# unilight/seq2seq-vc

Hardware: AMD Instinct MI355X
Metric: mel-frames/sec (train) (higher is better)
Workload: dtype bf16; 1 GPU; VTN egs/arctic/vc1 (vtn.v1.yaml) training step: fwd+Seq2SeqLoss+bwd+clip+Adam+WarmupLR; batch_per_gpu=32, global_batch=32, T_src=256, T_tgt=256, mel_dim=80, parallelism=dp1, split_backward=False, hip_graph=True, backward_stages=1

## Files before the change

include/s2svc_hip.h:

```cpp
#ifndef S2SVC_HIP_H
#define S2SVC_HIP_H
#include <stdint.h>
#ifdef __cplusplus
extern "C" {
#endif

const char* s2svc_last_error(void);
int s2svc_abi_version(void);
int s2svc_launch_floor(int workgroups, int threads, void* sink_1024_words, void* stream);

int s2svc_event_create(void** out );
int s2svc_event_destroy(void* ev);
int s2svc_event_record(void* ev, void* stream);
int s2svc_stream_wait_event(void* stream, void* ev);

enum { S2SVC_LAYOUT_KC = 0,
       S2SVC_LAYOUT_RC = 1 };
enum { S2SVC_OP_DENSE = 0,
       S2SVC_OP_CONV1D = 1,
       S2SVC_OP_CONV2D_S2 = 2,
       S2SVC_OP_TCONV2D_S2 = 3 };

typedef struct {
  const void* ptr;
// ... 18 lines not shown
  const void* res;
  int64_t ldr, rbs0, rbs1;
  int32_t M, N, K;
  int32_t nb0, nb1;
  int32_t act;
  float alpha;
  int32_t dtype;
  int32_t accumulate;
  int32_t splitk;
  float* ws;
  float* a_rowsum;
  float* a_rowsum_ws;
  int32_t a_rowsum_accumulate;
  int32_t tile_hint;
  const void* emask;
  int64_t ldm;
  float drop_p;
  int32_t emask_mode;
  const uint64_t* seed_base;
  uint64_t seed_off;
  int32_t c_map;
  int32_t cm_T1, cm_F1, cm_Tc, cm_Fc, cm_pt, cm_pf;
  int32_t reserved3_;
  void* c_pre;
} s2svc_gemm_desc;

int s2svc_gemm(const s2svc_gemm_desc* desc , void* stream);
const char* s2svc_gemm_last_route(void);

int s2svc_tconv2d_weights(int O, int C, const float* w, void* out_bf16, void* stream);

int s2svc_gemm_grouped_ok(const s2svc_gemm_desc* desc );
int s2svc_gemm_grouped(const s2svc_gemm_desc* descs , int n, int tile, void* stream);
int s2svc_gemm_grouped_batched(const s2svc_gemm_desc* descs , int n, void* stream);
int s2svc_gemm_wgrad_ok(const s2svc_gemm_desc* desc );
int64_t s2svc_gemm_wgrad_ws_floats(const s2svc_gemm_desc* descs , int n);
int s2svc_gemm_wgrad_grouped(const s2svc_gemm_desc* descs , int n, float* ws, void* stream);
int s2svc_gemm_wgrad_grouped_bg(const s2svc_gemm_desc* descs , int n, float* ws, void* stream, int wgs_cap);
int s2svc_gemm_set_w8(int on, int kt_chunk);

int s2svc_gemm_set_8ph(int mode);

int s2svc_layernorm_fwd(int dtype, int rows, int D, const void* x, const void* res, float drop_p, float hscale,
                        const uint64_t* seed_base, uint64_t seed_off, const float* gamma, const float* beta, float eps,
                        void* y, void* s_out, float* mean, float* rstd, void* stream);
int s2svc_layernorm_bwd(int dtype, int rows, int D, const void* dy, const void* s, const float* mean, const float* rstd,
                        const float* gamma, const void* ds_extra, float drop_p, float hscale, const uint64_t* seed_base,
                        uint64_t seed_off, void* ds, void* dh, void* stream);
int s2svc_colreduce(int dtype, int rows, int D, int mode, const void* dy, const void* x, const float* mean,
                    const float* rstd, float scale, float* out_sum, float* out_dot, int accumulate, float* ws,
                    int ws_chunks, int Tn, const int32_t* vlens , void* stream);
typedef struct {
  const void* dy;
  const void* x;
  const float* mean;
  const float* rstd;
  float* out_sum;
  float* out_dot;
  float* ws;
  int32_t dtype, rows, D, mode, accumulate, ws_chunks;
  float scale;
  int32_t reserved_;
} s2svc_colreduce_item;
int s2svc_colreduce_grouped(const s2svc_colreduce_item* items , int n, void* stream);
int s2svc_layernorm_bwd_pg_chunks(int dtype, int rows, int D, const void* dy, const void* s, const float* gamma, const void* ds_extra,
                                  const void* ds, const void* dh);
// ... 374 lines not shown
```

seq2seq_vc_amd/csrc/gemm_8ph.hip:

```cpp
#include <cstring>
#include "gemm_common.h"
#include "lds_dma.h"

namespace {

enum { P8_DENSE = 0, P8_CONV2D = 1, P8_TCONV2D = 2, P8_CONV1D = 3 };

template <int BM, int BN, bool GROUPED = false>
__device__ __forceinline__ void p8_tile_of_block(int& bm, int& bn) {
  const int gx = gridDim.x, gy = gridDim.y, nwg = gx * gy;
  int id = blockIdx.y * gx + blockIdx.x;
  if (gridDim.z == 1 || (nwg & 7) == 0) id = xcd_contiguous_id(id, nwg);
  if (GROUPED && gx >= 4) {
    const int qe = (nwg >> 3) < 32 ? (nwg >> 3) : 32;
    const int t2 = 2 * qe * BN / BM;
    int gh = 1;
    while (gh * 2 <= gy && 4 * gh * gh <= t2) gh *= 2;
    const int per = gh * gx, grp = id / per, within = id - grp * per;
    const int rows = (gy - grp * gh) < gh ? (gy - grp * gh) : gh;
    const int c = within / rows;
    bm = grp * gh + (within - c * rows);
    bn = c;
    return;
  }
  bm = id / gx;
  bn = id - bm * gx;
}

template <int KIND>
struct P8Walk {
  int kt, c0, kh, kw;
  __device__ __forceinline__ void init(const s2svc_operand& o, int kt0) {
    kt = kt0;
    if (KIND == P8_CONV1D) {
      const int ntap = 2 * o.pad + 1;
      const int cs = kt0 / ntap;
      c0 = cs * 64;
      kh = kt0 - cs * ntap;
      kw = 0;
    }
    if (KIND == P8_CONV2D) {
      const int cs = kt0 / 9, tap = kt0 - cs * 9;
      c0 = cs * 64;
      kh = tap / 3;
      kw = tap - kh * 3;
    }
    if (KIND == P8_TCONV2D) {
      const int nf = 2 - (o.pad & 1), ntap = (2 - (o.pad >> 1)) * nf;
      const int cs = kt0 / ntap, tap = kt0 - cs * ntap;
      c0 = cs * 64;
      kh = tap / nf;
      kw = tap - kh * nf;
    }
  }
  __device__ __forceinline__ int64_t off_bytes(const s2svc_operand& o) const {
    if (KIND == P8_CONV2D) return ((int64_t)(kh * o.F1 + kw) * o.ld + c0) * 2;
    if (KIND == P8_TCONV2D) return (-(int64_t)(kh * o.F2 + kw) * o.ld + c0) * 2;
    if (KIND == P8_CONV1D) return ((int64_t)(kh - o.pad) * o.ld + c0) * 2;
    return (int64_t)kt * 128;
  }
  __device__ __forceinline__ int64_t off_bytes_b(const s2svc_operand& o) const {
    if (KIND == P8_CONV2D) return ((int64_t)(kh * 3 + kw) * o.C + c0) * 2;
    if (KIND == P8_TCONV2D) return ((int64_t)(kh * (2 - (o.pad & 1)) + kw) * o.C + c0) * 2;
    if (KIND == P8_CONV1D) return ((int64_t)kh * o.C + c0) * 2;
    return (int64_t)kt * 128;
  }
  __device__ __forceinline__ int bit() const { return KIND == P8_CONV1D ? 1 << kh : 1 << (2 * kh + kw); }
  __device__ __forceinline__ void next(const s2svc_operand& o) {
    ++kt;
    if (KIND == P8_CONV2D) {
      if (++kw == 3) {
        kw = 0;
        if (++kh == 3) {
          kh = 0;
          c0 += 64;
        }
      }
    }
    if (KIND == P8_CONV1D) {
      if (++kh == 2 * o.pad + 1) {
        kh = 0;
        c0 += 64;
      }
    }
    if (KIND == P8_TCONV2D) {
      if (++kw == 2 - (o.pad & 1)) {
        kw = 0;
        if (++kh == 2 - (o.pad >> 1)) {
          kh = 0;
          c0 += 64;
        }
      }
    }
  }
};

template <int KIND>
__device__ __forceinline__ uint32_t p8_rowoff(const s2svc_operand& o, int r, int R, int c) {
  if (r >= R) r = R - 1;
  int64_t e;
  if (KIND == P8_CONV2D) {
    const int bt = r / o.F2, f2 = r - bt * o.F2;
    const int b = bt / o.T2, t2 = bt - b * o.T2;
    e = ((int64_t)(b * o.T1 + 2 * t2) * o.F1 + 2 * f2) * o.ld;
  } else if (KIND == P8_TCONV2D) {
    const int per_b = o.T1 * o.F1;
    const int b = r / per_b, rem = r - b * per_b;
    const int i = rem / o.F1, j = rem - i * o.F1;
    e = ((int64_t)(b * o.T2 + i) * o.F2 + j) * o.ld;
  } else {
    e = (int64_t)r * o.ld;
  }
  return (uint32_t)((e + c * 8) * 2);
}

__device__ __forceinline__ int p8_rowmask(const s2svc_operand& o, int r, int R) {
  if (r >= R) return 0;
  const int per_b = o.T1 * o.F1;
  const int rem = r - (r / per_b) * per_b;
  const int i = rem / o.F1, j = rem - i * o.F1;
  int m = 0;
#pragma unroll
  for (int ta = 0; ta < 2; ++ta)
#pragma unroll
    for (int fb = 0; fb < 2; ++fb)
      if (i - ta >= 0 && i - ta < o.T2 && j - fb >= 0 && j - fb < o.F2) m |= 1 << (2 * ta + fb);
  return m;
}

__device__ __forceinline__ int p8_rowmask1d(const s2svc_operand& o, int r, int R) {
  if (r >= R) return 0;
  const int t = r - (r / o.T) * o.T;
  int m = 0;
  for (int tap = 0; tap <= 2 * o.pad; ++tap)
    if (t + tap - o.pad >= 0 && t + tap - o.pad < o.T) m |= 1 << tap;
  return m;
}
template <int KA>
__device__ __forceinline__ int p8_rowmask_of(const s2svc_operand& o, int r, int R) {
  return KA == P8_TCONV2D ? p8_rowmask(o, r, R) : KA == P8_CONV1D ? p8_rowmask1d(o, r, R) : 0;
}

template <int NI>
__device__ __forceinline__ void p8_issue(const char* base, const uint32_t (&off)[NI], char* lds_unit, int wave_s) {
  const char* b = base ? base : reinterpret_cast<const char*>(&g_zero16);
#pragma unroll
  for (int e = 0; e < NI; ++e) {
    const uint32_t o = base ? off[e] : 0u;
    __builtin_amdgcn_global_load_lds((gbl_void*)(b + o), (lds_void*)(lds_unit + (wave_s * NI + e) * 1024), 16, 0, 0);
  }
}

template <int NI>
__device__ __forceinline__ void p8_issue_masked(const char* base, const uint32_t (&off)[NI], const int (&mask)[NI], int bit,
                                                char* lds_unit, int wave_s) {
  const char* z = reinterpret_cast<const char*>(&g_zero16);
#pragma unroll
  for (int e = 0; e < NI; ++e) {
    const char* src = (base && (mask[e] & bit)) ? base + off[e] : z;
    __builtin_amdgcn_global_load_lds((gbl_void*)src, (lds_void*)(lds_unit + (wave_s * NI + e) * 1024), 16, 0, 0);
  }
}

template <int KA, int NI>
__device__ __forceinline__ void p8_issue_a(const char* base, const uint32_t (&off)[NI], const int (&mask)[NI], int bit, char* lds_unit,
                                           int wave_s) {
  if (KA == P8_TCONV2D || KA == P8_CONV1D) p8_issue_masked<NI>(base, off, mask, bit, lds_unit, wave_s);
  else p8_issue<NI>(base, off, lds_unit, wave_s);
}

template <int NF>
__device__ __forceinline__ void p8_read(const char* unit, int rd_base, int p0, int p1, bf16x8_t (&f)[NF][2]) {
#pragma unroll
  for (int i = 0; i < NF; ++i) {
    f[i][0] = *reinterpret_cast<const bf16x8_t*>(unit + rd_base + i * 2048 + p0);
    f[i][1] = *reinterpret_cast<const bf16x8_t*>(unit + rd_base + i * 2048 + p1);
  }
}

template <int NA, int NB>
__device__ __forceinline__ void p8_mfma(const bf16x8_t (&a)[NA][2], const bf16x8_t (&b)[NB][2], f32x4_t (&acc)[NA][NB]) {
  __builtin_amdgcn_s_setprio(1);
#pragma unroll
  for (int ks = 0; ks < 2; ++ks)
#pragma unroll
    for (int i = 0; i < NA; ++i)
#pragma unroll
      for (int j = 0; j < NB; ++j) acc[i][j] = __builtin_amdgcn_mfma_f32_16x16x32_bf16(a[i][ks], b[j][ks], acc[i][j], 0, 0, 0);
  __builtin_amdgcn_s_setprio(0);
}

#define P8_PHASE_SYNC_IN()                 \
  wait_lgkm0();                         \
  __builtin_amdgcn_sched_barrier(0);       \
  __builtin_amdgcn_s_barrier();            \
  __builtin_amdgcn_sched_barrier(0)
#define P8_PHASE_SYNC_OUT()                \
  __builtin_amdgcn_sched_barrier(0);       \
  __builtin_amdgcn_s_barrier();            \
  __builtin_amdgcn_sched_barrier(0)

template <int KA, int WR, int WC, bool STAGGER, bool LEAN = false>
__global__ __launch_bounds__(512) void gemm_8ph_kernel_q(const s2svc_gemm_desc d) {
  static_assert(WR * WC == 8 && (WC == 2 || WC == 4), "8 waves");
  constexpr int BM = WR * 128, BN = WC * 64;
  constexpr int NIA = WR, NIB = WC / 2;
  constexpr int UA = WR * 64 * 128, UB = WC * 32 * 128;
  constexpr int BUF = 2 * UA + 2 * UB;
  constexpr int OA0 = 0, OA1 = UA, OB0 = 2 * UA, OB1 = 2 * UA + UB;
  __shared__ __attribute__((aligned(1024))) char smem[2 * BUF];
  const int zb = blockIdx.z;
  const int z0 = zb / d.nb1, z1 = zb - z0 * d.nb1;
  int tile_m, tile_n;
  p8_tile_of_block<BM, BN, true>(tile_m, tile_n);
  const int m0 = tile_m * BM, n0 = tile_n * BN;
  const char* Ab = reinterpret_cast<const char*>((const bf16_t*)d.A.ptr + (int64_t)z0 * d.A.bs0 + (int64_t)z1 * d.A.bs1);
  const char* Bb = reinterpret_cast<const char*>((const bf16_t*)d.B.ptr + (int64_t)z0 * d.B.bs0 + (int64_t)z1 * d.B.bs1);
  const int nt = d.K / 64;
  const int lane = threadIdx.x & 63;
  const int wave = __builtin_amdgcn_readfirstlane(threadIdx.x >> 6);
  const int wr = wave / WC, wc = wave % WC;
  const int half = wave >> 2;
  const int lr = lane & 15, lg = lane >> 4;

  uint32_t offA[2][NIA], offB[2][NIB];
  int mA[2][NIA];
#pragma unroll
  for (int e = 0; e < NIA; ++e) {
    const int ru = (wave * NIA + e) * 8 + (lane >> 3);
    const int c = (lane & 7) ^ ((ru >> 1) & 7);
#pragma unroll
    for (int h = 0; h < 2; ++h) {
      const int row = m0 + (ru >> 6) * 128 + h * 64 + (ru & 63);
      offA[h][e] = p8_rowoff<KA>(d.A, row, d.M, c);
      mA[h][e] = p8_rowmask_of<KA>(d.A, row, d.M);
    }
  }
#pragma unroll
  for (int e = 0; e < NIB; ++e) {
    const int ru = (wave * NIB + e) * 8 + (lane >> 3);
    const int c = (lane & 7) ^ ((ru >> 1) & 7);
#pragma unroll
    for (int h = 0; h < 2; ++h) offB[h][e] = p8_rowoff<P8_DENSE>(d.B, n0 + (ru >> 5) * 64 + h * 32 + (ru & 31), d.N, c);
  }
  const int sw = (lr >> 1) & 7;
  const int p0 = (lg ^ sw) << 4, p1 = ((4 + lg) ^ sw) << 4;
  const int rdA = (wr * 64 + lr) * 128, rdB = (wc * 32 + lr) * 128;
// ... 39 lines not shown
    char* oth = smem + ((t & 1) ^ 1) * BUF;
    const char* a2 = (t + 2 < nt) ? Ab + wa.off_bytes(d.A) : nullptr;
    const int bit2 = wa.bit();
    const char* b2 = (t + 2 < nt) ? Bb + wa.off_bytes_b(d.A) : nullptr;
    const char* b1 = (t + 1 < nt) ? Bb + wb.off_bytes_b(d.A) : nullptr;
    p8_read<2>(cur + OB0, rdB, p0, p1, fb0);
    p8_read<4>(cur + OA0, rdA, p0, p1, fa);
    p8_issue<NIB>(b1, offB[0], oth + OB0, wave);
    P8_PHASE_SYNC_IN();
    p8_mfma<4, 2>(fa, fb0, acc[0][0]);
    P8_PHASE_SYNC_OUT();
    p8_read<2>(cur + OB1, rdB, p0, p1, fb1);
    p8_issue_a<KA, NIA>(a2, offA[0], mA[0], bit2, cur + OA0, wave);
    P8_PHASE_SYNC_IN();
    p8_mfma<4, 2>(fa, fb1, acc[0][1]);
    P8_PHASE_SYNC_OUT();
    p8_read<4>(cur + OA1, rdA, p0, p1, fa);
    p8_issue<NIB>(b2, offB[1], cur + OB1, wave);
    P8_PHASE_SYNC_IN();
    p8_mfma<4, 2>(fa, fb1, acc[1][1]);
    P8_PHASE_SYNC_OUT();
    p8_issue_a<KA, NIA>(a2, offA[1], mA[1], bit2, cur + OA1, wave);
    wait_vmcnt<2 * NIA + NIB>();
    P8_PHASE_SYNC_IN();
    p8_mfma<4, 2>(fa, fb0, acc[1][0]);
    P8_PHASE_SYNC_OUT();
    wa.next(d.A);
    wb.next(d.A);
  }
  if (STAGGER && half == 0) __builtin_amdgcn_s_barrier();
  wait_vmcnt<0>();
  __syncthreads();
  float* cs = reinterpret_cast<float*>(smem) + wave * (64 * 32);
  const bool cmap_lean = KA == P8_TCONV2D && d.tile_hint != 65 && epilogue_cmap_ok(d);
  const c_map_t cmq = c_map_make(d);
#pragma unroll 1
  for (int q = 0; q < 4; ++q) {
    switch (q) {
      case 0: epilogue_stage<64, 32>(acc[0][0], cs); break;
      case 1: epilogue_stage<64, 32>(acc[0][1], cs); break;
      case 2: epilogue_stage<64, 32>(acc[1][0], cs); break;
      default: epilogue_stage<64, 32>(acc[1][1], cs); break;
    }
    if (LEAN) epilogue_flush_common<64, 32>(d, m0 + wr * 128 + (q >> 1) * 64, n0 + wc * 64 + (q & 1) * 32, cs);
    else if (KA == P8_TCONV2D && cmap_lean) epilogue_flush_cmap<64, 32>(d, cmq, m0 + wr * 128 + (q >> 1) * 64, n0 + wc * 64 + (q & 1) * 32, cs);
    else epilogue_flush<64, 32>(d, z0, z1, m0 + wr * 128 + (q >> 1) * 64, n0 + wc * 64 + (q & 1) * 32, cs, 1, 0, zb);
  }
}

template <int KA, bool STAGGER, int LEAN = 0>
__global__ __launch_bounds__(512) void gemm_8ph_kernel_128(const s2svc_gemm_desc d) {
  constexpr int UNIT = 16384, BUF = 3 * UNIT;
  __shared__ __attribute__((aligned(1024))) char smem[2 * BUF];
  const int zb = blockIdx.z;
  const int z0 = zb / d.nb1, z1 = zb - z0 * d.nb1;
  int tile_m, tile_n;
  p8_tile_of_block<256, 128>(tile_m, tile_n);
  const int m0 = tile_m * 256, n0 = tile_n * 128;
  const char* Ab = reinterpret_cast<const char*>((const bf16_t*)d.A.ptr + (int64_t)z0 * d.A.bs0 + (int64_t)z1 * d.A.bs1);
  const char* Bb = reinterpret_cast<const char*>((const bf16_t*)d.B.ptr + (int64_t)z0 * d.B.bs0 + (int64_t)z1 * d.B.bs1);
  const int nt = d.K / 64;
  const int lane = threadIdx.x & 63;
  const int wave = __builtin_amdgcn_readfirstlane(threadIdx.x >> 6);
  const int wr = wave >> 2, wc = wave & 3;
  const int lr = lane & 15, lg = lane >> 4;

  uint32_t offA[2][2], offB[2];
  int mA[2][2];
#pragma unroll
  for (int e = 0; e < 2; ++e) {
    const int ru = (wave * 2 + e) * 8 + (lane >> 3);
    const int c = (lane & 7) ^ ((ru >> 1) & 7);
#pragma unroll
    for (int h = 0; h < 2; ++h) {
      const int row = m0 + (ru >> 6) * 128 + h * 64 + (ru & 63);
      offA[h][e] = p8_rowoff<KA>(d.A, row, d.M, c);
      mA[h][e] = p8_rowmask_of<KA>(d.A, row, d.M);
    }
// ... 819 lines not shown
    if (md >= 2) { if (md == 2 || md == 2 + ph) return ph; continue; }
    if (t <= 256 && t >= 224 && (geo == 0 || tiles < 224 || tiles > 256)) return ph;
  }
  return 0;
}

int g_p8_geo = -1;
int p8_force_bn() {
  if (g_p8_geo < 0) g_p8_geo = 0;
  return g_p8_geo;
}

bool p8_operand_ok(const s2svc_operand& o, int rows, int K) {
  if (o.layout != S2SVC_LAYOUT_KC || ((uintptr_t)o.ptr) % 16 || o.ld % 8 || o.bs0 % 8 || o.bs1 % 8) return false;
  int64_t elems;
  if (o.mode == S2SVC_OP_DENSE) {
    elems = (int64_t)rows * o.ld;
  } else if (o.mode == S2SVC_OP_CONV2D_S2) {
    if (o.C % 64 || o.C < 64 || K != 9 * o.C) return false;
    elems = (int64_t)(rows / (o.T2 * o.F2) + 1) * o.T1 * o.F1 * o.ld;
  } else if (o.mode == S2SVC_OP_CONV1D) {
    if (o.pad < 0 || o.pad > 7 || o.C % 64 || o.C < 64 || K != (2 * o.pad + 1) * o.C || o.T <= 0 || rows % o.T || o.ld < o.C) return false;
    elems = (int64_t)(rows + o.pad) * o.ld;
  } else if (o.mode == S2SVC_OP_TCONV2D_S2) {
    const int ntap = (2 - (o.pad >> 1)) * (2 - (o.pad & 1));
    if (o.pad < 0 || o.pad > 3 || o.C % 64 || o.C < 64 || K != ntap * o.C || o.T1 <= 0 || o.F1 <= 0) return false;
    elems = (int64_t)(rows / (o.T1 * o.F1) + 1) * o.T2 * o.F2 * o.ld;
  } else {
    return false;
  }
  return elems * 2 < (1ll << 32);
}

}

extern "C" int s2svc_gemm_set_8ph(int mode) {
  const int prev = p8_mode() | (p8_force_bn() << 4) | ((p8_n96_mode() + 1) << 8);
  if (mode >= 0) {
    const int n96 = (mode >> 8) & 15;
    mode &= 255;
    if ((mode & 15) <= 2 && (mode >> 4) <= 3) {
      g_p8_mode = mode & 15;
      g_p8_geo = mode >> 4;
    }
    if (n96 >= 1 && n96 <= 6) g_p8_n96 = n96 - 1;
  }
  return prev;
}

extern "C" int s2svc_gemm_try_8ph(const s2svc_gemm_desc* desc, void* stream) {
  const s2svc_gemm_desc& d = *desc;
  const int mode = p8_mode();
  if (mode != 0 && d.tile_hint != 64 && p8_tr_ok(d) && (int64_t)(d.M / 256) * (d.N / 128) >= p8_min_tiles()) {
    const int64_t t128 = (int64_t)(d.M / 256) * (d.N / 128);
    if (p8_tr_take_q(d.N % 256 == 0, t128 / 2, t128)) {
      dim3 grid((unsigned)(d.N / 256), (unsigned)(d.M / 256), 1);
      s2s_gemm_route(mode == 2 ? "8ph_tr_q<noskew>" : "8ph_tr_q<skew>");
      if (mode == 2) hipLaunchKernelGGL((gemm_8ph_tr_kernel_q<false>), grid, dim3(512), 0, (hipStream_t)stream, d);
      else hipLaunchKernelGGL((gemm_8ph_tr_kernel_q<true>), grid, dim3(512), 0, (hipStream_t)stream, d);
    } else {
      dim3 grid((unsigned)(d.N / 128), (unsigned)(d.M / 256), 1);
      s2s_gemm_route(mode == 2 ? "8ph_tr<noskew>" : "8ph_tr<skew>");
      if (mode == 2) hipLaunchKernelGGL((gemm_8ph_tr_kernel<false>), grid, dim3(512), 0, (hipStream_t)stream, d);
      else hipLaunchKernelGGL((gemm_8ph_tr_kernel<true>), grid, dim3(512), 0, (hipStream_t)stream, d);
    }
    S2S_CHECK_LAUNCH("gemm_8ph_tr_kernel");
    return 1;
  }
  if (mode == 0 || d.dtype != S2S_BF16 || d.splitk > 1 || d.a_rowsum || d.tile_hint == 64) return 0;
  if (d.K < 128 || d.K % 64 || d.M < 256 || d.N < 64) return 0;
  if (d.B.mode != S2SVC_OP_DENSE || !p8_operand_ok(d.A, d.M, d.K) || !p8_operand_ok(d.B, d.N, d.K)) return 0;
  if (d.A.mode == S2SVC_OP_TCONV2D_S2 && d.nb0 * d.nb1 != 1) return 0;
  const int64_t nb = (int64_t)d.nb0 * d.nb1;
  const int64_t t256 = (int64_t)((d.M + 255) / 256) * ((d.N + 255) / 256) * nb;
  const int64_t t512 = (int64_t)((d.M + 511) / 512) * ((d.N + 127) / 128) * nb;
  const int64_t t128 = (int64_t)((d.M + 255) / 256) * ((d.N + 127) / 128) * nb;
  int geo = 0;
  const int waste256 = (int)(((d.N + 255) / 256) * 256 - d.N), waste128 = (int)(((d.N + 127) / 128) * 128 - d.N);
  const double cost256 = 2.0 * 0.85 * (double)((t256 + 255) / 256), cost128 = (double)((t128 + 255) / 256);
  if (waste256 <= waste128 && t256 >= 192 && cost256 <= cost128) geo = 1;
  else if (d.M >= 2048 && t512 >= 160 && t512 <= 256) geo = 2;
  else if (t128 >= p8_min_tiles()) geo = 3;
  if (p8_force_bn() >= 1 && p8_force_bn() <= 3) geo = p8_force_bn();
  hipStream_t st = (hipStream_t)stream;
  if (d.A.mode == S2SVC_OP_DENSE && nb == 1 && mode == 1 && (p8_force_bn() == 0 || p8_n96_mode() >= 2) && epilogue_common_ok(d)) {
    const int ph = p8_n96_phases(d, geo, geo == 1 ? t256 : geo == 2 ? t512 : t128);
    if (ph) {
      dim3 grid((unsigned)((d.N + 96 * ph - 1) / (96 * ph)), (unsigned)((d.M + 255) / 256), 1);
      s2s_gemm_route(ph == 3 ? "8ph_n96<3>" : "8ph_n96<2>");
      if (ph == 3) hipLaunchKernelGGL((gemm_8ph_kernel_n96<3, true>), grid, dim3(512), 0, st, d);
      else hipLaunchKernelGGL((gemm_8ph_kernel_n96<2, true>), grid, dim3(512), 0, st, d);
      S2S_CHECK_LAUNCH("gemm_8ph_kernel_n96");
      return 1;
    }
  }
  if (geo == 0) return 0;
  if (d.A.mode == S2SVC_OP_CONV1D) {
    if (mode != 1 || nb != 1 || !epilogue_common_ok(d)) return 0;
    const int bm1 = geo == 2 ? 512 : 256, bn1 = geo == 1 ? 256 : 128;
    dim3 grid1((unsigned)((d.N + bn1 - 1) / bn1), (unsigned)((d.M + bm1 - 1) / bm1), 1);
    s2s_gemm_route(geo == 1 ? "8ph_q<CONV1D,2,4>" : geo == 2 ? "8ph_q<CONV1D,4,2>" : "8ph_128<CONV1D,lean>");
    if (geo == 1) hipLaunchKernelGGL((gemm_8ph_kernel_q<P8_CONV1D, 2, 4, true, true>), grid1, dim3(512), 0, st, d);
    else if (geo == 2) hipLaunchKernelGGL((gemm_8ph_kernel_q<P8_CONV1D, 4, 2, true, true>), grid1, dim3(512), 0, st, d);
    else hipLaunchKernelGGL((gemm_8ph_kernel_128<P8_CONV1D, true, 1>), grid1, dim3(512), 0, st, d);
    S2S_CHECK_LAUNCH("gemm_8ph_kernel (conv1d)");
    return 1;
  }
  const bool conv = d.A.mode == S2SVC_OP_CONV2D_S2, tconv = d.A.mode == S2SVC_OP_TCONV2D_S2;
  const int bm = geo == 2 ? 512 : 256, bn = geo == 1 ? 256 : 128;
  dim3 grid((unsigned)((d.N + bn - 1) / bn), (unsigned)((d.M + bm - 1) / bm), (unsigned)nb);
#define P8_LAUNCH(PRE, POST, KERNEL, ...)                                                                   \
  do {                                                                                                    \
    s2s_gemm_route(mode == 2 ? (conv ? PRE "CONV2D" POST ",noskew>" : tconv ? PRE "TCONV2D" POST ",noskew>" : PRE "DENSE" POST ",noskew>")    \
                             : (conv ? PRE "CONV2D" POST ",skew>" : tconv ? PRE "TCONV2D" POST ",skew>" : PRE "DENSE" POST ",skew>"));        \
    if (mode == 2) {                                                                                      \
      if (conv) hipLaunchKernelGGL((KERNEL<P8_CONV2D, ##__VA_ARGS__, false>), grid, dim3(512), 0, st, d); \
      else if (tconv) hipLaunchKernelGGL((KERNEL<P8_TCONV2D, ##__VA_ARGS__, false>), grid, dim3(512), 0, st, d); \
      else hipLaunchKernelGGL((KERNEL<P8_DENSE, ##__VA_ARGS__, false>), grid, dim3(512), 0, st, d);       \
    } else {                                                                                              \
// ... 24 lines not shown
  group_args g;
  std::memset(&g, 0, sizeof(g));
  int64_t t128 = 0, t256 = 0;
  bool all256 = true;
  int mask = 0, m = 0;
  for (int i = 0; i < n; ++i) {
    if (!p8_tr_ok(descs[i]) || (int64_t)(descs[i].M / 128) * (descs[i].N / 128) < 64) continue;
    mask |= 1 << i;
    g.d[m++] = descs[i];
    t128 += (int64_t)(descs[i].M / 256) * (descs[i].N / 128);
    all256 = all256 && descs[i].N % 256 == 0;
    t256 += (int64_t)(descs[i].M / 256) * (descs[i].N / 256);
  }
  if (m == 0) return 0;
  S2S_REQUIRE(t128 < (1ll << 30), "gemm_grouped: too many tiles");
  g.n = m;
  const bool q = p8_tr_take_q(all256, t256, t128);
  int64_t total = 0;
  for (int i = 0; i < m; ++i) {
    g.tile_start[i] = (int32_t)total;
    total += (int64_t)(g.d[i].M / 256) * (g.d[i].N / (q ? 256 : 128));
  }
  for (int i = m; i <= GROUP_MAX; ++i) g.tile_start[i] = (int32_t)total;
  hipStream_t st = (hipStream_t)stream;
  if (q) {
    if (mode == 2) hipLaunchKernelGGL((gemm_8ph_tr_grouped_kernel<false, 256>), dim3((unsigned)total), dim3(512), 0, st, g);
    else hipLaunchKernelGGL((gemm_8ph_tr_grouped_kernel<true, 256>), dim3((unsigned)total), dim3(512), 0, st, g);
  } else {
    if (mode == 2) hipLaunchKernelGGL((gemm_8ph_tr_grouped_kernel<false, 128>), dim3((unsigned)total), dim3(512), 0, st, g);
    else hipLaunchKernelGGL((gemm_8ph_tr_grouped_kernel<true, 128>), dim3((unsigned)total), dim3(512), 0, st, g);
  }
  S2S_CHECK_LAUNCH("gemm_8ph_tr_grouped_kernel");
  return mask;
}

namespace {
int g_w8_mode = -1, g_w8_kt = -1;
int w8_mode() {
  if (g_w8_mode < 0) g_w8_mode = 1;
  return g_w8_mode;
}
int w8_kt_chunk_env() {
  if (g_w8_kt < 0) g_w8_kt = 64;
  return g_w8_kt;
}
constexpr int W8_CONV_KT_CHUNK = 75;
void w8_chunks(int M, int N, int K, int& nchunks, int& kt_chunk, bool conv = false) {
  const int ktiles = (K + 63) / 64;
  if (conv) {
    kt_chunk = W8_CONV_KT_CHUNK;
    nchunks = (ktiles + kt_chunk - 1) / kt_chunk;
    return;
  }
  if ((int64_t)((M + 255) / 256) * ((N + 127) / 128) >= 64) {
    nchunks = 1;
    kt_chunk = ktiles;
    return;
  }
  kt_chunk = w8_kt_chunk_env();
  nchunks = (ktiles + kt_chunk - 1) / kt_chunk;
  if (nchunks > 16) {
    kt_chunk = (ktiles + 15) / 16;
    nchunks = (ktiles + kt_chunk - 1) / kt_chunk;
  }
}
bool w8_ok(const s2svc_gemm_desc& d) {
// ... 120 lines not shown
```

seq2seq_vc_amd/ops/functional.py:

```python
import math
import os

import torch
from torch.autograd import Function

from . import kernels as K
from . import kernels_attn as KAT

_STATE = {"dtype": torch.float32}


def set_compute_dtype(dtype):
    if dtype not in (torch.float32, torch.bfloat16):
        raise ValueError("compute dtype must be float32 or bfloat16")
    _STATE["dtype"] = dtype


def compute_dtype():
    return _STATE["dtype"]


def to_compute(x):
    return K.cast(x.contiguous(), _STATE["dtype"])

# ... 1289 lines not shown
            if _slotted(weight, bias):
                _side_run(work, keep=(dy, x))
            else:
                dw, db = work()
        elif bias is not None and bias.requires_grad:
            db, _ = _reduce_to(bias, None, 0, dy.view(B * T, Cout))
        return dx, dw, db, None


class _CropRows(Function):

    @staticmethod
    def forward(ctx, x, vlens):
        from . import kernels_sdp as KS
        ctx.vlens = vlens
        return KS.mask_rows(_c(x), vlens)

    @staticmethod
    def backward(ctx, dy):
        from . import kernels_sdp as KS
        return KS.mask_rows(_c(dy), ctx.vlens), None


def crop_rows(x, vlens):
    return x if vlens is None else _CropRows.apply(x, vlens)


def conv1d(x, weight, bias=None, act=None, vlens=None):
    if vlens is not None and weight.shape[-1] > 1:
        x = crop_rows(x, vlens)
    return _Conv1d.apply(x, weight, bias, act)






class _Conv2dS2(Function):
    @staticmethod
    def forward(ctx, x, weight, bias, grad_premasked=False, input_is_relu=False):
        x = _c(x)
        ctx.grad_premasked = grad_premasked
        ctx.input_is_relu = input_is_relu
        B, T1, F1, C = x.shape
        O = weight.shape[0]
        T2, F2 = (T1 - 3) // 2 + 1, (F1 - 3) // 2 + 1
        dtype = x.dtype
        wp = K.gather3_cached(weight, (O, 9, C), (C * 9, 1, 9), 0, dtype)
        y = torch.empty((B, T2, F2, O), dtype=dtype, device=x.device)
        K.gemm(K.operand(x, C, mode=K.CONV2D_S2, C=C, T1=T1, F1=F1, T2=T2, F2=F2), K.operand(wp, 9 * C), B * T2 * F2, O, 9 * C, y,
               in_dtype=dtype, bias=bias, act="relu")
        ctx.params = (weight, bias)
        ctx.save_for_backward(x, y, wp)
        return y

    @staticmethod
    def backward(ctx, dy):
        x, y, wp = ctx.saved_tensors
        weight, bias = ctx.params
        B, T1, F1, C = x.shape
        O = weight.shape[0]
        T2, F2 = y.shape[1], y.shape[2]
        M2 = B * T2 * F2
        dtype = x.dtype
        dy = _c(dy) if ctx.grad_premasked else K.act_dropout_bwd(_c(dy), y, act="relu")
        dw = db = None
        if weight.requires_grad:
            def work():
                dwp = torch.empty((O, 9 * C), dtype=torch.float32, device=x.device)
                rs, racc, dbv = _bias_sink(bias, O)
                tile, sk = K.plan_gemm(O, 9 * C, M2)
                K.gemm(K.operand(dy, O, layout=K.RC),
                       K.operand(x, C, layout=K.RC, mode=K.CONV2D_S2, C=C, T1=T1, F1=F1, T2=T2, F2=F2), O, 9 * C, M2, dwp,
                       in_dtype=dtype, splitk=sk, tile=tile, a_rowsum=rs, a_rowsum_accumulate=racc, wgrad=True)
                return _emit_permuted(weight, dwp, O, 9, C), dbv
            if _slotted(weight, bias):
                _side_run(work, keep=(dy, x))
                _side_flush()
            else:
                dw, db = work()
        dx = None
        if ctx.needs_input_grad[0] and dtype == torch.bfloat16 and O % 8 == 0 and O >= 64 and C % 8 == 0:
            wts = K.tconv2d_weights_cached(weight)
            dx = torch.empty((B, T1, F1, C), dtype=dtype, device=x.device)
            mask = x if ctx.input_is_relu else None
            for cls, wt in enumerate(wts):
                pt, pf = cls >> 1, cls & 1
                Tc, Fc = (T1 - pt + 1) // 2, (F1 - pf + 1) // 2
                if Tc <= 0 or Fc <= 0:
                    continue
                Kc = wt.shape[1]
                K.gemm(K.operand(dy, O, mode=K.TCONV2D_S2, C=O, T1=Tc, F1=Fc, T2=T2, F2=F2, pad=cls), K.operand(wt, Kc),
                       B * Tc * Fc, C, Kc, dx, in_dtype=dtype, c_map=(T1, F1, Tc, Fc, pt, pf), emask=mask)
        elif ctx.needs_input_grad[0]:
            dcols = torch.empty((M2, 9 * C), dtype=dtype, device=x.device)
            K.gemm(K.operand(dy, O), K.operand(wp, 9 * C, layout=K.RC), M2, 9 * C, O, dcols, in_dtype=dtype)
            dx = K.col2im_s2(dcols, B, T1, F1, C, T2, F2)
            if ctx.input_is_relu:
                dx = K.act_dropout_bwd(dx, x, act="relu")
        if not weight.requires_grad and bias is not None and bias.requires_grad:
            db, _ = _reduce_to(bias, None, 0, dy.view(M2, O))
        return dx, dw, db, None, None


def conv2d_s2_relu(x_nhwc, weight, bias, grad_premasked=False, input_is_relu=False):
    return _Conv2dS2.apply(x_nhwc, weight, bias, grad_premasked, input_is_relu)


class _ConvIn1(Function):

    @staticmethod
    def forward(ctx, x, weight, bias, grad_premasked=False):
        x = _c(x)
        y = K.conv_in1_fwd(x, weight.detach(), bias.detach() if bias is not None else None)
        ctx.params = (weight, bias)
        ctx.grad_premasked = grad_premasked
        ctx.save_for_backward(x, y)
        return y

    @staticmethod
    def backward(ctx, dy):
        x, y = ctx.saved_tensors
        weight, bias = ctx.params
        dy = _c(dy)
        ym = None if ctx.grad_premasked else y
        wslot, bslot = getattr(weight, "_s2s_grad", None), getattr(bias, "_s2s_grad", None) if bias is not None else None
# ... 269 lines not shown
```

seq2seq_vc_amd/ops/kernels.py:

```python
import ctypes
import math
import os

import torch

from .. import _lib

KC, RC = 0, 1
DENSE, CONV1D, CONV2D_S2, TCONV2D_S2 = 0, 1, 2, 3
ACT = {None: 0, "none": 0, "relu": 1, "tanh": 2, "swish": 3, "sigmoid": 4, "gelu": 5}

_DT = {torch.float32: 0, torch.bfloat16: 1}


def dt(t):
    try:
        return _DT[t.dtype if isinstance(t, torch.Tensor) else t]
    except KeyError:
        raise TypeError(f"unsupported dtype {t.dtype if isinstance(t, torch.Tensor) else t}")


def ptr(t):
    return None if t is None else t.data_ptr()

# ... 402 lines not shown
        self.prev, _CR_RECORDER = _CR_RECORDER, self.queue
        return self.queue

    def __exit__(self, *exc):
        global _CR_RECORDER
        _CR_RECORDER = self.prev
        return False


def flush_colreduce(queue):
    pending = list(queue)
    del queue[:]
    while pending:
        seen, group, rest = set(), [], []
        for it, keep in pending:
            keys = {it.out_sum} | ({it.out_dot} if it.out_dot else set())
            if keys & seen:
                rest.append((it, keep))
            else:
                seen |= keys
                group.append((it, keep))
        pending = rest
        arr = (_lib.ColreduceItem * len(group))(*[g[0] for g in group])
        if _Audit.on:
            _audit_write("grouped column reduction", *[g[0].out_sum for g in group], *[g[0].out_dot for g in group])
        _lib.check(_lib.lib().s2svc_colreduce_grouped(ctypes.addressof(arr), len(group), stream()), "s2svc_colreduce_grouped")


def launch_group(descs, tile=128):
    arr = (_lib.GemmDesc * len(descs))(*descs)
    _lib.check(_lib.lib().s2svc_gemm_grouped(ctypes.addressof(arr), len(descs), tile, stream()), "s2svc_gemm_grouped")


_W8_CAP = [0]


def set_wgrad_cap(wgs):
    _W8_CAP[0] = max(0, int(wgs))


def get_wgrad_cap():
    return _W8_CAP[0]


def launch_wgrad_group(descs, capped=True):
    L = _lib.lib()
    arr = (_lib.GemmDesc * len(descs))(*descs)
    nws = L.s2svc_gemm_wgrad_ws_floats(ctypes.addressof(arr), len(descs))
    ws = torch.empty(nws, dtype=torch.float32, device=torch.cuda.current_device()) if nws else None
    if capped and _W8_CAP[0] > 0:
        _lib.check(L.s2svc_gemm_wgrad_grouped_bg(ctypes.addressof(arr), len(descs), ptr(ws), stream(), _W8_CAP[0]),
                   "s2svc_gemm_wgrad_grouped_bg")
        return
    _lib.check(L.s2svc_gemm_wgrad_grouped(ctypes.addressof(arr), len(descs), ptr(ws), stream()), "s2svc_gemm_wgrad_grouped")


def launch_group_batched(descs):
    if not descs:
        return
    if len(descs) > 1:
        arr = (_lib.GemmDesc * len(descs))(*descs)
        rc = _lib.lib().s2svc_gemm_grouped_batched(ctypes.addressof(arr), len(descs), stream())
        if rc == 0:
            return
        if rc != 1:
            _lib.check(rc, "s2svc_gemm_grouped_batched")
# ... 654 lines not shown
```

Measured before the change: 1.747 million mel-frames/sec.

## Group the four transposed-conv parity-class dgrad GEMMs into one persistent launch

The input-gradient of the stride-2 conv was computed as up to four separate parity-class GEMM launches. These are now collected as descriptors and run in a single grouped 8-phase kernel. Work units are ordered by K (largest first) and swizzled per segment so tiles from all classes share one grid. A tap-major K-iteration variant is added for classes that don't qualify for the normal 8-phase geometry. The aim is to cut launch count and fill the GPU better on small per-class problems, at the cost of a larger kernel argument struct and extra index math per block.

```diff
diff --git a/include/s2svc_hip.h b/include/s2svc_hip.h
--- a/include/s2svc_hip.h
+++ b/include/s2svc_hip.h
@@ -74,6 +74,9 @@
 
 int s2svc_gemm_grouped_ok(const s2svc_gemm_desc* desc );
 int s2svc_gemm_grouped(const s2svc_gemm_desc* descs , int n, int tile, void* stream);
+int s2svc_tconv2d_grouped_ok(const s2svc_gemm_desc* descs , int n);
+int s2svc_tconv2d_grouped_units(const s2svc_gemm_desc* descs , int n, int32_t* units , int cap);
+int s2svc_tconv2d_grouped(const s2svc_gemm_desc* descs , int n, void* stream);
 int s2svc_gemm_grouped_batched(const s2svc_gemm_desc* descs , int n, void* stream);
 int s2svc_gemm_wgrad_ok(const s2svc_gemm_desc* desc );
 int64_t s2svc_gemm_wgrad_ws_floats(const s2svc_gemm_desc* descs , int n);
diff --git a/seq2seq_vc_amd/csrc/gemm_8ph.hip b/seq2seq_vc_amd/csrc/gemm_8ph.hip
--- a/seq2seq_vc_amd/csrc/gemm_8ph.hip
+++ b/seq2seq_vc_amd/csrc/gemm_8ph.hip
@@ -1,10 +1,12 @@
 #include <cstring>
+#include <utility>
 #include "gemm_common.h"
 #include "lds_dma.h"
 
 namespace {
 
-enum { P8_DENSE = 0, P8_CONV2D = 1, P8_TCONV2D = 2, P8_CONV1D = 3 };
+enum { P8_DENSE = 0, P8_CONV2D = 1, P8_TCONV2D = 2, P8_CONV1D = 3, P8_TCONV2D_TM = 4 };
+constexpr bool p8_is_tconv(int kind) { return kind == P8_TCONV2D || kind == P8_TCONV2D_TM; }
 
 template <int BM, int BN, bool GROUPED = false>
 __device__ __forceinline__ void p8_tile_of_block(int& bm, int& bn) {
@@ -52,16 +54,23 @@
       kh = tap / nf;
       kw = tap - kh * nf;
     }
+    if (KIND == P8_TCONV2D_TM) {
+      const int nf = 2 - (o.pad & 1), ns = o.C / 64;
+      const int tap = kt0 / ns;
+      c0 = (kt0 - tap * ns) * 64;
+      kh = tap / nf;
+      kw = tap - kh * nf;
+    }
   }
   __device__ __forceinline__ int64_t off_bytes(const s2svc_operand& o) const {
     if (KIND == P8_CONV2D) return ((int64_t)(kh * o.F1 + kw) * o.ld + c0) * 2;
-    if (KIND == P8_TCONV2D) return (-(int64_t)(kh * o.F2 + kw) * o.ld + c0) * 2;
+    if (p8_is_tconv(KIND)) return (-(int64_t)(kh * o.F2 + kw) * o.ld + c0) * 2;
     if (KIND == P8_CONV1D) return ((int64_t)(kh - o.pad) * o.ld + c0) * 2;
     return (int64_t)kt * 128;
   }
   __device__ __forceinline__ int64_t off_bytes_b(const s2svc_operand& o) const {
     if (KIND == P8_CONV2D) return ((int64_t)(kh * 3 + kw) * o.C + c0) * 2;
-    if (KIND == P8_TCONV2D) return ((int64_t)(kh * (2 - (o.pad & 1)) + kw) * o.C + c0) * 2;
+    if (p8_is_tconv(KIND)) return ((int64_t)(kh * (2 - (o.pad & 1)) + kw) * o.C + c0) * 2;
     if (KIND == P8_CONV1D) return ((int64_t)kh * o.C + c0) * 2;
     return (int64_t)kt * 128;
   }
@@ -92,6 +101,16 @@
         }
       }
     }
+    if (KIND == P8_TCONV2D_TM) {
+      c0 += 64;
+      if (c0 == o.C) {
+        c0 = 0;
+        if (++kw == 2 - (o.pad & 1)) {
+          kw = 0;
+          ++kh;
+        }
+      }
+    }
   }
 };
 
@@ -103,7 +122,7 @@
     const int bt = r / o.F2, f2 = r - bt * o.F2;
     const int b = bt / o.T2, t2 = bt - b * o.T2;
     e = ((int64_t)(b * o.T1 + 2 * t2) * o.F1 + 2 * f2) * o.ld;
-  } else if (KIND == P8_TCONV2D) {
+  } else if (p8_is_tconv(KIND)) {
     const int per_b = o.T1 * o.F1;
     const int b = r / per_b, rem = r - b * per_b;
     const int i = rem / o.F1, j = rem - i * o.F1;
@@ -138,7 +157,7 @@
 }
 template <int KA>
 __device__ __forceinline__ int p8_rowmask_of(const s2svc_operand& o, int r, int R) {
-  return KA == P8_TCONV2D ? p8_rowmask(o, r, R) : KA == P8_CONV1D ? p8_rowmask1d(o, r, R) : 0;
+  return p8_is_tconv(KA) ? p8_rowmask(o, r, R) : KA == P8_CONV1D ? p8_rowmask1d(o, r, R) : 0;
 }
 
 template <int NI>
@@ -165,7 +184,7 @@
 template <int KA, int NI>
 __device__ __forceinline__ void p8_issue_a(const char* base, const uint32_t (&off)[NI], const int (&mask)[NI], int bit, char* lds_unit,
                                            int wave_s) {
-  if (KA == P8_TCONV2D || KA == P8_CONV1D) p8_issue_masked<NI>(base, off, mask, bit, lds_unit, wave_s);
+  if (p8_is_tconv(KA) || KA == P8_CONV1D) p8_issue_masked<NI>(base, off, mask, bit, lds_unit, wave_s);
   else p8_issue<NI>(base, off, lds_unit, wave_s);
 }
 
@@ -200,19 +219,52 @@
   __builtin_amdgcn_s_barrier();            \
   __builtin_amdgcn_sched_barrier(0)
 
-template <int KA, int WR, int WC, bool STAGGER, bool LEAN = false>
-__global__ __launch_bounds__(512) void gemm_8ph_kernel_q(const s2svc_gemm_desc d) {
+constexpr int TCONV_CLASSES = 4;
+struct tconv_group_args {
+  s2svc_gemm_desc d[TCONV_CLASSES];
+  int32_t seg_start[TCONV_CLASSES + 1];
+  int32_t gx[TCONV_CLASSES];
+  int32_t n;
+};
+
+__host__ __device__ inline void tconv_unit(const int32_t* seg_start, const int32_t* gx, int n, int u, int& p, int& tile_m, int& tile_n) {
+  p = 0;
+  for (int i = 1; i < TCONV_CLASSES; ++i) p += (i < n && seg_start[i] <= u) ? 1 : 0;
+  const int s8 = seg_start[p] & 7, run = 8 * gx[p];
+  int v = u - seg_start[p] + s8;
+  const int base = v / run * run;
+  if (base >= s8 && base + run <= seg_start[p + 1] - seg_start[p] + s8) v = base + (v & 7) * gx[p] + ((v - base) >> 3);
+  v -= s8;
+  tile_m = v / gx[p];
+  tile_n = v - tile_m * gx[p];
+}
+
+template <class ARGS> struct P8Args;
+template <> struct P8Args<s2svc_gemm_desc> {
+  static constexpr bool UNITS = false;
+  static __device__ __forceinline__ const s2svc_gemm_desc& problem(const s2svc_gemm_desc& d, int) { return d; }
+};
+template <> struct P8Args<tconv_group_args> {
+  static constexpr bool UNITS = true;
+  static __device__ __forceinline__ const s2svc_gemm_desc& problem(const tconv_group_args& g, int p) { return g.d[p]; }
+};
+
+template <int KA, int WR, int WC, bool STAGGER, bool LEAN = false, class ARGS = s2svc_gemm_desc>
+__global__ __launch_bounds__(512) void gemm_8ph_kernel_q(const ARGS args) {
   static_assert(WR * WC == 8 && (WC == 2 || WC == 4), "8 waves");
+  constexpr bool UNITS = P8Args<ARGS>::UNITS;
   constexpr int BM = WR * 128, BN = WC * 64;
   constexpr int NIA = WR, NIB = WC / 2;
   constexpr int UA = WR * 64 * 128, UB = WC * 32 * 128;
   constexpr int BUF = 2 * UA + 2 * UB;
   constexpr int OA0 = 0, OA1 = UA, OB0 = 2 * UA, OB1 = 2 * UA + UB;
   __shared__ __attribute__((aligned(1024))) char smem[2 * BUF];
-  const int zb = blockIdx.z;
+  int unit_p = 0, tile_m, tile_n;
+  if constexpr (UNITS) tconv_unit(args.seg_start, args.gx, args.n, (int)blockIdx.x, unit_p, tile_m, tile_n);
+  const s2svc_gemm_desc& d = P8Args<ARGS>::problem(args, unit_p);
+  const int zb = UNITS ? 0 : blockIdx.z;
   const int z0 = zb / d.nb1, z1 = zb - z0 * d.nb1;
-  int tile_m, tile_n;
-  p8_tile_of_block<BM, BN, true>(tile_m, tile_n);
+  if constexpr (!UNITS) p8_tile_of_block<BM, BN, true>(tile_m, tile_n);
   const int m0 = tile_m * BM, n0 = tile_n * BN;
   const char* Ab = reinterpret_cast<const char*>((const bf16_t*)d.A.ptr + (int64_t)z0 * d.A.bs0 + (int64_t)z1 * d.A.bs1);
   const char* Bb = reinterpret_cast<const char*>((const bf16_t*)d.B.ptr + (int64_t)z0 * d.B.bs0 + (int64_t)z1 * d.B.bs1);
@@ -318,7 +370,7 @@
   wait_vmcnt<0>();
   __syncthreads();
   float* cs = reinterpret_cast<float*>(smem) + wave * (64 * 32);
-  const bool cmap_lean = KA == P8_TCONV2D && d.tile_hint != 65 && epilogue_cmap_ok(d);
+  const bool cmap_lean = p8_is_tconv(KA) && d.tile_hint != 65 && epilogue_cmap_ok(d);
   const c_map_t cmq = c_map_make(d);
 #pragma unroll 1
   for (int q = 0; q < 4; ++q) {
@@ -329,7 +381,7 @@
       default: epilogue_stage<64, 32>(acc[1][1], cs); break;
     }
     if (LEAN) epilogue_flush_common<64, 32>(d, m0 + wr * 128 + (q >> 1) * 64, n0 + wc * 64 + (q & 1) * 32, cs);
-    else if (KA == P8_TCONV2D && cmap_lean) epilogue_flush_cmap<64, 32>(d, cmq, m0 + wr * 128 + (q >> 1) * 64, n0 + wc * 64 + (q & 1) * 32, cs);
+    else if (p8_is_tconv(KA) && cmap_lean) epilogue_flush_cmap<64, 32>(d, cmq, m0 + wr * 128 + (q >> 1) * 64, n0 + wc * 64 + (q & 1) * 32, cs);
     else epilogue_flush<64, 32>(d, z0, z1, m0 + wr * 128 + (q >> 1) * 64, n0 + wc * 64 + (q & 1) * 32, cs, 1, 0, zb);
   }
 }
@@ -1215,6 +1267,26 @@
   return elems * 2 < (1ll << 32);
 }
 
+int p8_kc_geo(const s2svc_gemm_desc& d, int64_t* tiles) {
+  if (p8_mode() == 0 || d.dtype != S2S_BF16 || d.splitk > 1 || d.a_rowsum || d.tile_hint == 64) return -1;
+  if (d.K < 128 || d.K % 64 || d.M < 256 || d.N < 64) return -1;
+  if (d.B.mode != S2SVC_OP_DENSE || !p8_operand_ok(d.A, d.M, d.K) || !p8_operand_ok(d.B, d.N, d.K)) return -1;
+  if (d.A.mode == S2SVC_OP_TCONV2D_S2 && d.nb0 * d.nb1 != 1) return -1;
+  const int64_t nb = (int64_t)d.nb0 * d.nb1;
+  const int64_t t256 = (int64_t)((d.M + 255) / 256) * ((d.N + 255) / 256) * nb;
+  const int64_t t512 = (int64_t)((d.M + 511) / 512) * ((d.N + 127) / 128) * nb;
+  const int64_t t128 = (int64_t)((d.M + 255) / 256) * ((d.N + 127) / 128) * nb;
+  int geo = 0;
+  const int waste256 = (int)(((d.N + 255) / 256) * 256 - d.N), waste128 = (int)(((d.N + 127) / 128) * 128 - d.N);
+  const double cost256 = 2.0 * 0.85 * (double)((t256 + 255) / 256), cost128 = (double)((t128 + 255) / 256);
+  if (waste256 <= waste128 && t256 >= 192 && cost256 <= cost128) geo = 1;
+  else if (d.M >= 2048 && t512 >= 160 && t512 <= 256) geo = 2;
+  else if (t128 >= p8_min_tiles()) geo = 3;
+  if (p8_force_bn() >= 1 && p8_force_bn() <= 3) geo = p8_force_bn();
+  if (tiles) *tiles = geo == 1 ? t256 : geo == 2 ? t512 : t128;
+  return geo;
+}
+
 }
 
 extern "C" int s2svc_gemm_set_8ph(int mode) {
@@ -1250,24 +1322,13 @@
     S2S_CHECK_LAUNCH("gemm_8ph_tr_kernel");
     return 1;
   }
-  if (mode == 0 || d.dtype != S2S_BF16 || d.splitk > 1 || d.a_rowsum || d.tile_hint == 64) return 0;
-  if (d.K < 128 || d.K % 64 || d.M < 256 || d.N < 64) return 0;
-  if (d.B.mode != S2SVC_OP_DENSE || !p8_operand_ok(d.A, d.M, d.K) || !p8_operand_ok(d.B, d.N, d.K)) return 0;
-  if (d.A.mode == S2SVC_OP_TCONV2D_S2 && d.nb0 * d.nb1 != 1) return 0;
+  int64_t geo_tiles = 0;
+  const int geo = p8_kc_geo(d, &geo_tiles);
+  if (geo < 0) return 0;
   const int64_t nb = (int64_t)d.nb0 * d.nb1;
-  const int64_t t256 = (int64_t)((d.M + 255) / 256) * ((d.N + 255) / 256) * nb;
-  const int64_t t512 = (int64_t)((d.M + 511) / 512) * ((d.N + 127) / 128) * nb;
-  const int64_t t128 = (int64_t)((d.M + 255) / 256) * ((d.N + 127) / 128) * nb;
-  int geo = 0;
-  const int waste256 = (int)(((d.N + 255) / 256) * 256 - d.N), waste128 = (int)(((d.N + 127) / 128) * 128 - d.N);
-  const double cost256 = 2.0 * 0.85 * (double)((t256 + 255) / 256), cost128 = (double)((t128 + 255) / 256);
-  if (waste256 <= waste128 && t256 >= 192 && cost256 <= cost128) geo = 1;
-  else if (d.M >= 2048 && t512 >= 160 && t512 <= 256) geo = 2;
-  else if (t128 >= p8_min_tiles()) geo = 3;
-  if (p8_force_bn() >= 1 && p8_force_bn() <= 3) geo = p8_force_bn();
   hipStream_t st = (hipStream_t)stream;
   if (d.A.mode == S2SVC_OP_DENSE && nb == 1 && mode == 1 && (p8_force_bn() == 0 || p8_n96_mode() >= 2) && epilogue_common_ok(d)) {
-    const int ph = p8_n96_phases(d, geo, geo == 1 ? t256 : geo == 2 ? t512 : t128);
+    const int ph = p8_n96_phases(d, geo, geo_tiles);
     if (ph) {
       dim3 grid((unsigned)((d.N + 96 * ph - 1) / (96 * ph)), (unsigned)((d.M + 255) / 256), 1);
       s2s_gemm_route(ph == 3 ? "8ph_n96<3>" : "8ph_n96<2>");
@@ -1358,6 +1419,80 @@
   }
   S2S_CHECK_LAUNCH("gemm_8ph_tr_grouped_kernel");
   return mask;
+}
+
+namespace {
+bool tconv8_desc_ok(const s2svc_gemm_desc& d) {
+  if (d.dtype != S2S_BF16 || d.c_dtype != S2S_BF16 || d.nb0 * d.nb1 > 1 || d.splitk > 1 || d.a_rowsum || d.res || d.drop_p != 0.f) return false;
+  if (d.A.mode != S2SVC_OP_TCONV2D_S2 || d.B.mode != S2SVC_OP_DENSE || !d.A.ptr || !d.B.ptr || !d.C) return false;
+  if (d.M <= 0 || d.N <= 0 || d.N % 8 || d.K < 64 || d.K % 64 || !p8_operand_ok(d.A, d.M, d.K) || !p8_operand_ok(d.B, d.N, d.K)) return false;
+  if (!d.c_map || d.cm_Tc <= 0 || d.cm_Fc <= 0 || d.M % (d.cm_Tc * d.cm_Fc)) return false;
+  if (d.emask && (d.emask_mode != 0 || d.ldm != d.ldc)) return false;
+  return true;
+}
+bool tconv8_plan(const s2svc_gemm_desc* descs, int n, tconv_group_args& g, int (&order)[TCONV_CLASSES], bool& tap_major) {
+  if (!descs || n < 1 || n > TCONV_CLASSES) return false;
+  int n8 = 0;
+  for (int i = 0; i < n; ++i) {
+    if (!tconv8_desc_ok(descs[i])) return false;
+    n8 += p8_kc_geo(descs[i], nullptr) > 0 ? 1 : 0;
+    order[i] = i;
+  }
+  if (n8 != 0 && n8 != n) return false;
+  tap_major = n8 == 0;
+  for (int i = 1; i < n; ++i)
+    for (int j = i; j > 0 && descs[order[j]].K > descs[order[j - 1]].K; --j) std::swap(order[j], order[j - 1]);
+  std::memset(&g, 0, sizeof(g));
+  g.n = n;
+  int64_t total = 0;
+  for (int i = 0; i < n; ++i) {
+    const s2svc_gemm_desc& d = descs[order[i]];
+    g.d[i] = d;
+    g.gx[i] = (d.N + 127) / 128;
+    g.seg_start[i] = (int32_t)total;
+    total += (int64_t)((d.M + 511) / 512) * g.gx[i];
+    if (total >= (1ll << 30)) return false;
+  }
+  for (int i = n; i <= TCONV_CLASSES; ++i) g.seg_start[i] = (int32_t)total;
+  return true;
+}
+}
+
+extern "C" int s2svc_tconv2d_grouped_ok(const s2svc_gemm_desc* descs, int n) {
+  tconv_group_args g;
+  int order[TCONV_CLASSES];
+  bool tm;
+  return tconv8_plan(descs, n, g, order, tm) ? 1 : 0;
+}
+
+extern "C" int s2svc_tconv2d_grouped_units(const s2svc_gemm_desc* descs, int n, int32_t* units, int cap) {
+  tconv_group_args g;
+  int order[TCONV_CLASSES];
+  bool tm;
+  S2S_REQUIRE(tconv8_plan(descs, n, g, order, tm), "tconv2d_grouped_units: the descriptors are not eligible (check s2svc_tconv2d_grouped_ok first)");
+  const int total = g.seg_start[TCONV_CLASSES];
+  for (int u = 0; u < total && u < cap && units; ++u) {
+    int p, tile_m, tile_n;
+    tconv_unit(g.seg_start, g.gx, g.n, u, p, tile_m, tile_n);
+    units[4 * u] = order[p];
+    units[4 * u + 1] = tile_m;
+    units[4 * u + 2] = tile_n;
+    units[4 * u + 3] = g.d[p].K / 64;
+  }
+  return total;
+}
+
+extern "C" int s2svc_tconv2d_grouped(const s2svc_gemm_desc* descs, int n, void* stream) {
+  tconv_group_args g;
+  int order[TCONV_CLASSES];
+  bool tm;
+  S2S_REQUIRE(tconv8_plan(descs, n, g, order, tm), "tconv2d_grouped: the descriptors are not eligible (check s2svc_tconv2d_grouped_ok first)");
+  const dim3 grid((unsigned)g.seg_start[TCONV_CLASSES]);
+  const auto gemm_grouped_tconv8 = tm ? gemm_8ph_kernel_q<P8_TCONV2D_TM, 4, 2, true, false, tconv_group_args>
+                                      : gemm_8ph_kernel_q<P8_TCONV2D, 4, 2, true, false, tconv_group_args>;
+  hipLaunchKernelGGL(gemm_grouped_tconv8, grid, dim3(512), 0, (hipStream_t)stream, g);
+  S2S_CHECK_LAUNCH("gemm_8ph_kernel_q (grouped transposed convolution)");
+  return 0;
 }
 
 namespace {
diff --git a/seq2seq_vc_amd/ops/functional.py b/seq2seq_vc_amd/ops/functional.py
--- a/seq2seq_vc_amd/ops/functional.py
+++ b/seq2seq_vc_amd/ops/functional.py
@@ -1345,8 +1345,7 @@
     return _Conv1d.apply(x, weight, bias, act)
 
 
-
-
+_NO_TCONV_GROUP = os.environ.get("S2SVC_NO_TCONV_GROUP", "0") == "1"
 
 
 class _Conv2dS2(Function):
@@ -1397,6 +1396,7 @@
             wts = K.tconv2d_weights_cached(weight)
             dx = torch.empty((B, T1, F1, C), dtype=dtype, device=x.device)
             mask = x if ctx.input_is_relu else None
+            descs = []
             for cls, wt in enumerate(wts):
                 pt, pf = cls >> 1, cls & 1
                 Tc, Fc = (T1 - pt + 1) // 2, (F1 - pf + 1) // 2
@@ -1404,7 +1404,12 @@
                     continue
                 Kc = wt.shape[1]
                 K.gemm(K.operand(dy, O, mode=K.TCONV2D_S2, C=O, T1=Tc, F1=Fc, T2=T2, F2=F2, pad=cls), K.operand(wt, Kc),
-                       B * Tc * Fc, C, Kc, dx, in_dtype=dtype, c_map=(T1, F1, Tc, Fc, pt, pf), emask=mask)
+                       B * Tc * Fc, C, Kc, dx, in_dtype=dtype, c_map=(T1, F1, Tc, Fc, pt, pf), emask=mask, group=descs)
+            if not _NO_TCONV_GROUP and K.tconv2d_grouped_ok(descs):
+                K.tconv2d_grouped(descs)
+            else:
+                for d in descs:
+                    K.gemm_desc(d)
         elif ctx.needs_input_grad[0]:
             dcols = torch.empty((M2, 9 * C), dtype=dtype, device=x.device)
             K.gemm(K.operand(dy, O), K.operand(wp, 9 * C, layout=K.RC), M2, 9 * C, O, dcols, in_dtype=dtype)
diff --git a/seq2seq_vc_amd/ops/kernels.py b/seq2seq_vc_amd/ops/kernels.py
--- a/seq2seq_vc_amd/ops/kernels.py
+++ b/seq2seq_vc_amd/ops/kernels.py
@@ -458,6 +458,30 @@
     _lib.check(_lib.lib().s2svc_gemm_grouped(ctypes.addressof(arr), len(descs), tile, stream()), "s2svc_gemm_grouped")
 
 
+def gemm_desc(d):
+    _lib.check(_lib.lib().s2svc_gemm(ctypes.byref(d), stream()), "s2svc_gemm")
+
+
+def tconv2d_grouped_ok(descs):
+    arr = (_lib.GemmDesc * len(descs))(*descs)
+    return bool(descs) and _lib.lib().s2svc_tconv2d_grouped_ok(ctypes.addressof(arr), len(descs)) == 1
+
+
+def tconv2d_grouped_units(descs):
+    arr = (_lib.GemmDesc * len(descs))(*descs)
+    n = _lib.lib().s2svc_tconv2d_grouped_units(ctypes.addressof(arr), len(descs), None, 0)
+    if n < 0:
+        _lib.check(n, "s2svc_tconv2d_grouped_units")
+    units = (ctypes.c_int32 * (4 * max(n, 1)))()
+    _lib.lib().s2svc_tconv2d_grouped_units(ctypes.addressof(arr), len(descs), ctypes.addressof(units), n)
+    return [tuple(units[4 * u:4 * u + 4]) for u in range(n)]
+
+
+def tconv2d_grouped(descs):
+    arr = (_lib.GemmDesc * len(descs))(*descs)
+    _lib.check(_lib.lib().s2svc_tconv2d_grouped(ctypes.addressof(arr), len(descs), stream()), "s2svc_tconv2d_grouped")
+
+
 _W8_CAP = [0]
 
 
```

After: 1.770 million mel-frames/sec (median of 5 runs). +1.3%, better.
